# AU-Master-Thesis/magics

Hardware: AMD Instinct MI355X
Metric: GBP iterations/sec (whole node), N robots x K horizon (higher is better)
Workload: dtype f64

## Files before the change

magics_amd/csrc/mgx_sweep.h:

```cpp
#pragma once
#include <hip/hip_runtime.h>

#include "gbp_math.h"
#include "mgx_dev.h"

namespace mgx {

constexpr int SWEEP_BLOCK = 128;
enum { ROLE_DYN = 0, ROLE_UV = 1 };
#ifndef MGX_WIDE
#define MGX_WIDE 0
#endif
template <int KT, bool PERSIST>
constexpr int sweep_waves() { return (MGX_WIDE && PERSIST && KT > 0 && 4 * KT <= 64) ? 4 : 2; }
template <int KT, bool PERSIST>
constexpr int sweep_threads() { return 64 * sweep_waves<KT, PERSIST>(); }

__device__ __forceinline__ void ld_soa4(const double *base, int stride, int item, double (&o)[4]) {
#pragma unroll
    for (int c = 0; c < 4; c++) o[c] = base[(size_t)c * stride + item];
}
__device__ __forceinline__ void ld_soa16(const double *base, int stride, int item, double (&o)[16]) {
#pragma unroll
    for (int c = 0; c < 16; c++) o[c] = base[(size_t)c * stride + item];
// ... 975 lines not shown
        }
        if (internal) {
#pragma unroll
            for (int c = 0; c < 4; c++) s_snap[(20 + c) * K + lane] = mu[c];
        }
    };

    auto quad_core = [&](const double *s_in, double *cov_img, bool &ok, bool &fin, double &mu_q) __attribute__((always_inline)) {
        const int q = lane / K, i = lane - q * K;
        double eta[4], lam[16];
#pragma unroll
        for (int c = 0; c < 4; c++) eta[c] = s_in[c * K + i];
#pragma unroll
        for (int c = 0; c < 16; c++) lam[c] = s_in[(4 + c) * K + i];
        bool not_zero = false;
#pragma unroll
        for (int c = 0; c < 16; c++) not_zero = not_zero || (lam[c] > 1e-6);
        double r0[4], r1[4], r2[4], mn[4], cf[4];
#pragma unroll
        for (int c = 0; c < 4; c++) {
            r0[c] = (q == 0) ? lam[4 + c] : lam[c];
            r1[c] = (q <= 1) ? lam[8 + c] : lam[4 + c];
            r2[c] = (q <= 2) ? lam[12 + c] : lam[8 + c];
        }
        minors_of_removed_row(r0, r1, r2, mn);
#pragma unroll
        for (int j = 0; j < 4; j++) cf[j] = ((q + j) & 1) ? -mn[j] : mn[j];
        const double row0[4] = {lam[0], lam[1], lam[2], lam[3]};
        const double det = __shfl(det_from_row0(row0, cf), i, 64);
        ok = not_zero && det != 0.0;
        const double id = 1.0 / det;
        double col[4];
        bool fin_own = true;
#pragma unroll
        for (int j = 0; j < 4; j++) {
            col[j] = cf[j] * id;
            fin_own = fin_own && std::isfinite(col[j]);
        }
        unsigned long long bad = __ballot(!fin_own);
        constexpr int KS = QUADFIN ? KT : 1;
        bad |= (bad >> KS) | (bad >> (2 * KS)) | (bad >> (3 * KS));
        fin = ((bad >> i) & 1ull) == 0ull;
        if (ok) {
#pragma unroll
            for (int j = 0; j < 4; j++) cov_img[(j * 4 + q) * K + i] = col[j];
            __builtin_amdgcn_wave_barrier();
            if (fin) {
                double cq[4];
#pragma unroll
                for (int c = 0; c < 4; c++) cq[c] = cov_img[(q * 4 + c) * K + i];
                mu_q = ((cq[0] * eta[0] + cq[1] * eta[1]) + cq[2] * eta[2]) + cq[3] * eta[3];
            }
        }
    };
    auto variable_finish_quad = [&](const double *s_in, bool internal) {
        const int q = lane / K, i = lane - q * K;
        double mu_q = s_mu[q * K + i];
        bool ok, fin;
        quad_core(s_in, s_cov, ok, fin, mu_q);
        if (ok) {
            if (fin) s_mu[q * K + i] = mu_q;
            if (q == 0) {
                s_valid[i] = fin ? 1 : 0;
                s_covset[i] = 1;
            }
        }
        if (internal) s_snap[(20 + q) * K + i] = mu_q;
    };
    auto finish = [&](const double *s_in, bool internal) __attribute__((always_inline)) {
        if constexpr (QUADFIN) {
            if (role == ROLE_UV && lane < 4 * K) variable_finish_quad(s_in, internal);
        } else {
            if (is_var) variable_finish(s_in, internal);
        }
    };

    auto dynamic_messages = [&](double *s_out) {
        double me[4], ml[16], oe[4], ol[16];
        const int o = dyn_other_var, oe_ix = dyn_other_edge;
        double paa[4], pab[4], pba[4], pbb[4];
        if (PERSIST) {
            load_dyn_potential(paa, pab, pba, pbb);
        } else {
#pragma unroll
            for (int c = 0; c < 4; c++) { paa[c] = maa[c]; pab[c] = mab[c]; pba[c] = mba[c]; pbb[c] = mbb[c]; }
        }
        if (s_epoch[o] > 0) {
#pragma unroll
            for (int c = 0; c < 4; c++) me[c] = s_snap[c * K + o] - s_fv[c * E1 + oe_ix];
#pragma unroll
            for (int c = 0; c < 16; c++) ml[c] = s_snap[(4 + c) * K + o] - s_fv[(4 + c) * E1 + oe_ix];
        } else {
#pragma unroll
            for (int c = 0; c < 4; c++) me[c] = 0.0;
#pragma unroll
            for (int c = 0; c < 16; c++) ml[c] = 0.0;
        }
        double me2[4], ml2[16];
        const int lane2 = lane + 64;
        const bool has2 = BIG && lane2 < n_dyn;
        if (has2) {
            const int f2 = lane2 % (K - 1), slot2 = lane2 / (K - 1), o2 = f2 + 1 - slot2, oe2 = (1 - slot2) * (K - 1) + f2;
            const bool pres = s_epoch[o2] > 0;
#pragma unroll
            for (int c = 0; c < 4; c++) me2[c] = pres ? s_snap[c * K + o2] - s_fv[c * E1 + oe2] : 0.0;
#pragma unroll
            for (int c = 0; c < 16; c++) ml2[c] = pres ? s_snap[(4 + c) * K + o2] - s_fv[(4 + c) * E1 + oe2] : 0.0;
        }
        if (!dynamic_message(paa, pab, pba, pbb, me, ml, oe, ol)) {
#pragma unroll
            for (int c = 0; c < 4; c++) oe[c] = 0.0;
#pragma unroll
            for (int c = 0; c < 16; c++) ol[c] = 0.0;
        }
#pragma unroll
        for (int c = 0; c < 4; c++) s_out[c * E1 + lane] = oe[c];
#pragma unroll
        for (int c = 0; c < 16; c++) s_out[(4 + c) * E1 + lane] = ol[c];
        if (has2) {
            const int f2 = lane2 % (K - 1), slot2 = lane2 / (K - 1), a2 = 2 * slot2, b2 = 2 * (1 - slot2), it2 = r * (K - 1) + f2;
            double naa[4], nab[4], nba[4], nbb[4];
#pragma unroll
            for (int i = 0; i < 2; i++)
#pragma unroll
                for (int j = 0; j < 2; j++) {
                    naa[i * 2 + j] = w.dyn_m[(size_t)((a2 + i) * 4 + (a2 + j)) * w.ND + it2];
                    nab[i * 2 + j] = w.dyn_m[(size_t)((a2 + i) * 4 + (b2 + j)) * w.ND + it2];
                    nba[i * 2 + j] = w.dyn_m[(size_t)((b2 + i) * 4 + (a2 + j)) * w.ND + it2];
                    nbb[i * 2 + j] = w.dyn_m[(size_t)((b2 + i) * 4 + (b2 + j)) * w.ND + it2];
                }
            if (!dynamic_message(naa, nab, nba, nbb, me2, ml2, oe, ol)) {
#pragma unroll
                for (int c = 0; c < 4; c++) oe[c] = 0.0;
#pragma unroll
                for (int c = 0; c < 16; c++) ol[c] = 0.0;
            }
#pragma unroll
            for (int c = 0; c < 4; c++) s_out[c * E1 + lane2] = oe[c];
#pragma unroll
            for (int c = 0; c < 16; c++) s_out[(4 + c) * E1 + lane2] = ol[c];
        }
    };

    const SdfView sdf = make_sdf_view(w.sdf, w.sdf_w, w.sdf_h, w.world_w, w.world_h);
    auto trk_pad_here = [&]() __attribute__((always_inline)) {
        double p_ = w.trk_pad;
        asm volatile("" : "+v"(p_));
        return p_;
    };
    auto obs_inv_delta_here = [&]() __attribute__((always_inline)) {
        double p_ = w.obs_inv_delta;
        asm volatile("" : "+s"(p_));
        return p_;
    };
    auto unary_messages = [&](uint32_t skip, double *s_out, int itf_gate) __attribute__((always_inline)) {
        if (obs_rows) {
            if (role == ROLE_UF && lane < 4 * (K - 2) && (w.enable & 4u) && !(skip & 4u)) {
                const int j = lane >> 2, q = lane & 3, var = j + 1, col = n_dyn + j;
                double x0[4];
                const bool pres = s_epoch[var] > 0;
#pragma unroll
                for (int c = 0; c < 4; c++) x0[c] = pres ? s_snap[(20 + c) * K + var] : 0.0;
                const long long idx = obstacle_tap(sdf, x0[0], x0[1], w.obs_delta, q);
                const double hq = (idx >= 0) ? sdf_value(w.sdf[idx]) : 0.0;
                double h[4];
#pragma unroll
                for (int t = 0; t < 4; t++) h[t] = __shfl(hq, (lane & ~3) + t, 64);
                double eta_q, lam_q[4];
                obstacle_message_row(h, w.obs_delta, obs_inv_delta_here(), w.inv_s2_obs, x0, q, eta_q, lam_q);
                s_out[q * E1 + col] = eta_q;
#pragma unroll
                for (int c = 0; c < 4; c++) s_out[(4 + q * 4 + c) * E1 + col] = lam_q[c];
            }
        } else if (is_obs && (w.enable & 4u) && !(skip & 4u)) {
            double x0[4], oe[4], ol[16];
            const bool pres = s_epoch[uvar] > 0;
#pragma unroll
            for (int c = 0; c < 4; c++) x0[c] = pres ? s_snap[(20 + c) * K + uvar] : 0.0;
            long long idx[4];
            obstacle_taps(sdf, x0[0], x0[1], w.obs_delta, idx);
            double h[4];
#pragma unroll
            for (int q = 0; q < 4; q++) h[q] = (idx[q] >= 0) ? sdf_value(w.sdf[idx[q]]) : 0.0;
            obstacle_message(h, w.obs_delta, obs_inv_delta_here(), w.inv_s2_obs, x0, oe, ol);
#pragma unroll
            for (int c = 0; c < 4; c++) s_out[c * E1 + uedge] = oe[c];
#pragma unroll
            for (int c = 0; c < 16; c++) s_out[(4 + c) * E1 + uedge] = ol[c];
        }
        if (is_trk && (w.enable & 8u) && itf_gate >= 10 && !(skip & 8u)) {
            double x0[4], oe[4], ol[16];
#pragma unroll
            for (int c = 0; c < 4; c++) x0[c] = s_snap[(20 + c) * K + uvar];
            const int p0 = w.path_ptr[r], np = w.path_ptr[r + 1] - p0;
            if (!tracking_update(w.path_xy + 2 * (size_t)p0, np, trk_pad_here(), w.trk_attr, w.inv_s2_trk, x0, trk_rec,
                                  trk_lp, trk_lv, oe, ol)) {
#pragma unroll
                for (int c = 0; c < 4; c++) oe[c] = 0.0;
#pragma unroll
                for (int c = 0; c < 16; c++) ol[c] = 0.0;
            }
#pragma unroll
            for (int c = 0; c < 4; c++) s_out[c * E1 + uedge] = oe[c];
#pragma unroll
            for (int c = 0; c < 16; c++) s_out[(4 + c) * E1 + uedge] = ol[c];
        }
        if (BIG && role == ROLE_UF && lane + 64 >= K - 2 && lane + 64 < 2 * (K - 2) && (w.enable & 8u) && itf_gate >= 10 &&
            !(skip & 8u)) {
            const int j2 = lane + 64 - (K - 2), var2 = j2 + 1, col2 = n_dyn + (K - 2) + j2, item2 = r * (K - 2) + j2;
            double x0[4], oe[4], ol[16];
#pragma unroll
            for (int c = 0; c < 4; c++) x0[c] = s_snap[(20 + c) * K + var2];
            int rec2 = w.trk_record[item2];
            float lp2[2] = {w.trk_last_pos[item2], w.trk_last_pos[(size_t)w.NT + item2]};
            double lv2 = w.trk_last_val[item2];
            const int p0 = w.path_ptr[r], np = w.path_ptr[r + 1] - p0;
            if (!tracking_update(w.path_xy + 2 * (size_t)p0, np, trk_pad_here(), w.trk_attr, w.inv_s2_trk, x0, rec2, lp2, lv2, oe, ol)) {
#pragma unroll
                for (int c = 0; c < 4; c++) oe[c] = 0.0;
#pragma unroll
                for (int c = 0; c < 16; c++) ol[c] = 0.0;
            }
            w.trk_record[item2] = rec2;
            w.trk_last_pos[item2] = lp2[0];
            w.trk_last_pos[(size_t)w.NT + item2] = lp2[1];
            w.trk_last_val[item2] = lv2;
#pragma unroll
            for (int c = 0; c < 4; c++) s_out[c * E1 + col2] = oe[c];
#pragma unroll
            for (int c = 0; c < 16; c++) s_out[(4 + c) * E1 + col2] = ol[c];
        }
    };

    int my_peer = -1, peer_q0 = 0, peer_q1 = 0;
    bool my_peer_read = false;
    if (PERSIST && radio && ir_on && role == ROLE_UV) {
        peer_q0 = w.peer_ptr[r];
        peer_q1 = w.peer_ptr[r + 1];
        if (peer_q0 + lane < peer_q1) {
            const int pr = w.peer_idx[peer_q0 + lane];
            if (w.antenna[pr] && !w.idle[pr]) my_peer = pr;
        }
        for (int e = w.ir_var_ptr[v0 + 1]; e < w.ir_var_ptr[v0 + 2]; e++) my_peer_read = my_peer_read || w.ir_rec[e].src_robot == my_peer;
    }
    auto progress_of = [&](int pr) __attribute__((always_inline)) {
        if (SHARD && pr >= w.R_local)
            return __hip_atomic_load(&cold().gflag[pr - w.R_local], __ATOMIC_RELAXED, __HIP_MEMORY_SCOPE_SYSTEM);
        return __hip_atomic_load(&w.sweep_flag[pr], __ATOMIC_RELAXED, __HIP_MEMORY_SCOPE_AGENT);
    };
    auto wait_for_progress = [&](unsigned long long want, bool ghosts_only) __attribute__((always_inline)) {
        if (PERSIST && radio && ir_on && role == ROLE_UV) {
            for (int q = peer_q0 + lane; q < peer_q1; q += 64) {
                int pr = my_peer;
                if (q != peer_q0 + lane) {
                    pr = w.peer_idx[q];
                    if (!w.antenna[pr] || w.idle[pr]) pr = -1;
                }
                if (pr < 0 || (ghosts_only && pr < w.R_local)) continue;
                if (!ghosts_only && q == peer_q0 + lane && my_peer_read) continue;
                const long long t0 = wall_clock64();
                unsigned spins = 0;
                while (progress_of(pr) < want) {
                    __builtin_amdgcn_s_sleep(4);
                    if ((++spins & 31u) == 0u) {
                        if (__hip_atomic_load(cold().sweep_abort, __ATOMIC_RELAXED, __HIP_MEMORY_SCOPE_AGENT) != 0ull) break;
                        if (wall_clock64() - t0 > cold_plan().timeout_ticks) {
                            const unsigned long long word = cold_plan().flag_base + 1ull;
                            __hip_atomic_store(cold().sweep_abort, word, __ATOMIC_RELAXED, __HIP_MEMORY_SCOPE_AGENT);
                            __hip_atomic_store(cold().sweep_err, word, __ATOMIC_RELAXED, __HIP_MEMORY_SCOPE_SYSTEM);
                            break;
                        }
                    }
                }
            }
        }
    };
    auto wait_for_peers = [&](int k) __attribute__((always_inline)) { wait_for_progress(plan.flag_base + (unsigned long long)k, false); };
    int xp0 = 0, xp1 = 0;
    if (SHARD && role == ROLE_UV) {
        xp0 = __builtin_amdgcn_readfirstlane(cold().xp_ptr[r]);
        xp1 = __builtin_amdgcn_readfirstlane(cold().xp_ptr[r + 1]);
    }

    bool prefired = false;
    bool par_done = false;
    bool pending = false;
    bool early = false;
    auto adopt_early = [&](int t0, int step) __attribute__((always_inline)) {
        for (int t = t0; t < 20 * E; t += step) {
            const int c = t / E, e = t - c * E;
            s_fv[c * E1 + e] = s_sh[c * E1 + e];
        }
    };
    int last_int_seg = -1, last_ext_seg = -1;
    int kbase = 0;
    if (PLDS && lane == 0) s_ps[0] = 0u;
    if (PLDS) __builtin_amdgcn_wave_barrier();
#ifdef MGX_STAMPS
    unsigned long long c_f = 0, c_fb = 0, c_v = 0, c_vb = 0, t_extf = t_staged, t_extv = t_staged, t_loop0 = t_staged;
    unsigned long long rt0 = __builtin_amdgcn_s_memrealtime();
    unsigned long long p_wait = 0, p_extf = 0, p_extv = 0, p_int = 0, p_pub = 0;
    unsigned long long qs[16] = {0, 0, 0, 0, 0, 0, 0, 0, 0, 0, 0, 0, 0, 0, 0, 0};
#define PSTAMP(v) const unsigned long long v = __builtin_readcyclecounter()
#define QSTAMP(i, since) do { const unsigned long long _n = __builtin_readcyclecounter(); qs[i] += _n - (since); (since) = _n; } while (0)
#define QBEGIN(v) unsigned long long v = __builtin_readcyclecounter()
#else
#define PSTAMP(v)
#define QSTAMP(i, since)
#define QBEGIN(v)
#endif
    for (int k = 0; PLDS || k < nseg; k++) {
        if (k == 0) {
            const int plans_done = PLDS ? (int)ps_word(0) : 0;
            const bool upd_now = PLDS ? plan_dword(1) != 0u : w.upd != nullptr;
            if (upd_now) {
                if constexpr (PLDS) {
#pragma unroll
                    for (int c = 0; c < 4; c++) u_rec[c] = s_urec[c];
                    u_bel = (lane < 20 && role < 2) ? s_tmp[4 * K + role * 20 + lane] : 0.0;
                }
                const double upd_max_speed = PLDS ? reinterpret_cast<const double *>(s_plan + 2 + MAX_SEGS / 2)[0] : w.upd_max_speed;
                const double upd_delta_t = PLDS ? reinterpret_cast<const double *>(s_plan + 2 + MAX_SEGS / 2)[1] : w.upd_delta_t;
                const uint32_t what = (uint32_t)u_rec[3];
                const int i = role == 0 ? K - 1 : 0;
                if (role < 2 && (role == 0 ? (what & 1u) : (what & 2u))) {
                    double m[4];
                    if (role == 0) {
                        const double ex = s_mu[0 * K + i], ey = s_mu[1 * K + i];
                        double hx = u_rec[0] - ex, hy = u_rec[1] - ey;
                        const double dist = std::sqrt(hx * hx + hy * hy);
                        double nx = hx, ny = hy;
                        if (!(dist == 0.0 || std::isinf(dist))) { nx = hx / dist; ny = hy / dist; }
                        const double sp = (upd_max_speed < dist || dist != dist) ? upd_max_speed : dist;
                        const double vx = sp * nx, vy = sp * ny;
                        m[0] = ex + vx * upd_delta_t; m[1] = ey + vy * upd_delta_t; m[2] = vx; m[3] = vy;
                    } else {
        #pragma unroll
                        for (int c = 0; c < 4; c++) {
                            const double m0 = s_mu[c * K + 0], m1 = s_mu[c * K + 1];
                            m[c] = m0 + u_rec[2] * (m1 - m0);
                        }
                    }
                    __builtin_amdgcn_wave_barrier();
                    if (lane < 4) {
                        double pl[4];
        #pragma unroll
                        for (int c = 0; c < 4; c++) pl[c] = s_prior[(4 + lane * 4 + c) * K + i];
                        const double pe = ((pl[0] * m[0] + pl[1] * m[1]) + pl[2] * m[2]) + pl[3] * m[3];
                        s_prior[lane * K + i] = pe;
                        blob[L.prior() + lane * K + i] = pe;
                    } else if (lane < 8) {
                        const double mc = lane == 4 ? m[0] : (lane == 5 ? m[1] : (lane == 6 ? m[2] : m[3]));
                        s_mu[(lane - 4) * K + i] = mc;
                        s_snap[(20 + lane - 4) * K + i] = mc;
                        if (PERSIST && have_xmu) s_xmu[(lane - 4) * K + i] = mc;
                    } else if (lane == 8) {
                        s_epoch[i] += 1;
                    }
                    if (lane < 20) s_snap[lane * K + i] = u_bel;
                    const int es[4] = {(i >= 1) ? (K - 1) + (i - 1) : -1, (i <= K - 2) ? i : -1,
                                       (i >= 1 && i <= K - 2) ? n_dyn + (i - 1) : -1, (i >= 1 && i <= K - 2) ? n_dyn + (K - 2) + (i - 1) : -1};
                    for (int t = lane; t < 80; t += 64) {
                        const int col = es[t & 3];
                        if (col >= 0) {
                            s_fv[(t >> 2) * E1 + col] = 0.0;
                            if (PERSIST) s_sh[(t >> 2) * E1 + col] = 0.0;
                        }
                    }
                    if (HAS_IR) {
                        const int x0 = w.ir_var_ptr[v0 + i], x1 = w.ir_var_ptr[v0 + i + 1];
                        for (int e = x0 + lane; e < x1; e += 64) {
                            if (w.enable & 2u) {
        #pragma unroll
                                for (int c = 0; c < 4; c++) w.ir_bmu[(size_t)c * w.NI + e] = m[c];
                            }
                            w.ir_fv_eta[0 * (size_t)w.NI + e] = 0.0;
                            w.ir_fv_eta[1 * (size_t)w.NI + e] = 0.0;
                            w.ir_fv_lam[0 * (size_t)w.NI + e] = 0.0;
                            w.ir_fv_lam[1 * (size_t)w.NI + e] = 0.0;
                            w.ir_fv_lam[4 * (size_t)w.NI + e] = 0.0;
                            w.ir_fv_lam[5 * (size_t)w.NI + e] = 0.0;
                            if (STAGE_IR) {
        #pragma unroll
                                for (int c = 0; c < 6; c++) s_ir[(e - ie0) * IR_STRIDE + c] = 0.0;
                            }
                        }
                    }
                }
                __syncthreads();
            }
            if (PERSIST && plans_done == 0) {
                for (int t = tid; t < 20 * E1; t += NT) s_sh[t] = s_fv[t];
                __syncthreads();
            }
            my_epoch = (sum_t < 4 * K) ? s_epoch[sum_t % K] : 0u;
            if constexpr (PLDS) {
                nseg = (int)plan_dword(0);
                const int q = lane & (MAX_SEGS - 1), q1 = (q + 1) & (MAX_SEGS - 1);
                auto byte_of = [&](int base, int i) __attribute__((always_inline)) { return (s_plan[base + (i >> 2)] >> (8 * (i & 3))) & 0xffu; };
                const uint32_t e_q = byte_of(2, q), n_q = byte_of(2 + MAX_SEGS / 4, q);
                const uint32_t e_1 = q + 1 < MAX_SEGS ? byte_of(2, q1) : 0u, n_1 = q + 1 < MAX_SEGS ? byte_of(2 + MAX_SEGS / 4, q1) : 0u;
                const bool in = lane < nseg;
                const unsigned long long m_int = __ballot(in && n_q > 0u), m_ext = __ballot(in && e_q != 0u);
                last_int_seg = m_int ? 63 - __clzll((long long)m_int) : -1;
                last_ext_seg = m_ext ? 63 - __clzll((long long)m_ext) : -1;
                has_int_var = m_int != 0ull && !idle;
                any_sweep = has_int_var || (m_ext != 0ull && radio);
                kbase = plans_done ? (int)ps_word(1) - 1 : 0;
                const bool lingers = LINGER && census && plan.linger_ticks > 0;
                if (lane < MAX_SEGS) {
                    const uint32_t bits = (e_q ? SEG_EXT : 0u) | (lane == nseg - 1 ? SEG_LAST : 0u) | (lane == last_int_seg ? SEG_LAST_INT : 0u) |
                                          (lane == last_ext_seg ? SEG_LAST_EXT : 0u) | ((lane == 0 && plans_done == 0) ? SEG_FIRST_OF_LAUNCH : 0u) |
                                          (lingers ? SEG_LINGERS : 0u);
                    s_seg[lane] = uint2{bits | (n_q << 8) | ((e_1 ? 1u : 0u) << 16) | (n_1 << 24), (uint32_t)(kbase + lane)};
                }
                __builtin_amdgcn_wave_barrier();
                if (lane == 0) {
                    s_ps[1] = (uint32_t)(kbase + nseg);
                    s_ps[2] = (has_int_var ? 1u : 0u) | (any_sweep ? 2u : 0u);
                }
                __builtin_amdgcn_wave_barrier();
            } else if (PERSIST) {
                bool plan_int = false, plan_has_ext = false;
                last_int_seg = last_ext_seg = -1;
                for (int q = 0; q < nseg; q++) {
                    if (plan_n_int(q) > 0) { plan_int = true; last_int_seg = q; }
                    if (plan_ext(q)) { plan_has_ext = true; last_ext_seg = q; }
                }
                has_int_var = plan_int && !idle;
                any_sweep = has_int_var || (plan_has_ext && radio);
            }
        }
        uint32_t seg_b = 0u;
        int kg = k;
        if constexpr (PLDS) {
            const uint2 e = s_seg[k];
            seg_b = (uint32_t)__builtin_amdgcn_readfirstlane((int)e.x);
            kg = __builtin_amdgcn_readfirstlane((int)e.y);
        } else if (PERSIST) {
            seg_b = (plan_ext(k) ? SEG_EXT : 0u) | ((uint32_t)plan_n_int(k) << 8) | (k == nseg - 1 ? SEG_LAST : 0u) | (k == last_int_seg ? SEG_LAST_INT : 0u) |
                    (k == last_ext_seg ? SEG_LAST_EXT : 0u) | (k == 0 ? SEG_FIRST_OF_LAUNCH : 0u);
            if (k + 1 < nseg) seg_b |= ((plan_ext(k + 1) ? 1u : 0u) << 16) | ((uint32_t)plan_n_int(k + 1) << 24);
        }
        const bool is_last_int_seg = (seg_b & SEG_LAST_INT) != 0u, is_last_ext_seg = (seg_b & SEG_LAST_EXT) != 0u;
        const bool lingers = LINGER && (seg_b & SEG_LINGERS) != 0u;
        if (PERSIST) asm volatile("" : "+v"(tid), "+v"(lane), "+v"(my_j), "+v"(pf_dst));
        const uint32_t ext_k = PERSIST ? ((seg_b & SEG_EXT) ? (PH_EXT_FACTOR | PH_EXT_VARIABLE) : 0u) : ext_mask;
        const uint32_t int_k = PERSIST ? (PH_INT_FACTOR | PH_INT_VARIABLE) : int_mask;
        const int n_int_k = PERSIST ? (int)((seg_b >> 8) & 0xffu) : n_int;
        const bool last_seg = PERSIST ? (seg_b & SEG_LAST) != 0u : true;
        PSTAMP(ps0);
        QBEGIN(qt);
        if (PERSIST && ext_k && k > 0) {
            wait_for_peers(kg);
            QSTAMP(0, qt);
            if (!(FUSED && par_done)) __syncthreads();
            QSTAMP(1, qt);
        }
        PSTAMP(ps1);
        if (ext_k & PH_EXT_FACTOR) {
            external_factor_sweep(k, kg, !PERSIST || is_last_ext_seg);
            QSTAMP(2, qt);
            __syncthreads();
            QSTAMP(3, qt);
        }
        PSTAMP(ps2);
#ifdef MGX_STAMPS
        if (k == 0) t_extf = __builtin_readcyclecounter();
#endif
        prefired = false;
        if constexpr (FUSED) {
            par_done = (ext_k & PH_EXT_VARIABLE) && radio && early && n_int_k == 1;
            if (par_done) {
                const bool is_last = is_last_int_seg && last_seg;
                const int q = lane / K, i = lane - q * K;
                bool ok_i = false, fin_i = false;
                double mu_i = 0.0;
                if (role == ROLE_UV) {
                    double *t_ = s_fv;
                    s_fv = s_sh;
                    s_sh = t_;
                    variable_sums(s_snap, true, false);
                    QSTAMP(4, qt);
                    if (lane < 4 * K) quad_core(s_snap, s_cov, ok_i, fin_i, mu_i);
                } else {
                    if (role == ROLE_DYN && lane < 4 * K) {
                        variable_sums_from(lane, 4 * K, s_tmp, false, false);
                        QSTAMP(4, qt);
                        double mu_x = s_mu[q * K + i];
                        bool ok_x, fin_x;
                        quad_core(s_tmp, s_tmp + 4 * K, ok_x, fin_x, mu_x);
                        s_xmu[q * K + i] = mu_x - 0.0;
                        if (q == 0) s_xok[i] = (ok_x ? 1 : 0) | (fin_x ? 2 : 0);
                    }
                    double *t_ = s_fv;
                    s_fv = s_sh;
                    s_sh = t_;
                }
                QSTAMP(6, qt);
                __syncthreads();
                QSTAMP(7, qt);
                DELAY_AT(5, true);
                if (role == ROLE_UV && lane < 4 * K) {
                    double mu_fin = mu_i;
                    const int xs = s_xok[i];
                    if (!(ok_i && fin_i)) {
                        mu_fin = s_xmu[q * K + i];
                        if (!ok_i && (xs & 1)) {
#pragma unroll
                            for (int j = 0; j < 4; j++) s_cov[(j * 4 + q) * K + i] = s_tmp[(4 + j * 4 + q) * K + i];
                        }
                    }
                    s_mu[q * K + i] = mu_fin;
                    s_snap[(20 + q) * K + i] = mu_fin;
                    if (is_last) {
                        s_prior[q * K + i] = s_snap[q * K + i];
#pragma unroll
                        for (int c = 0; c < 4; c++) s_prior[(4 + q * 4 + c) * K + i] = s_snap[(4 + q * 4 + c) * K + i];
                    }
                    if (q == 0) {
                        if (ok_i) {
                            s_valid[i] = fin_i ? 1 : 0;
                            s_covset[i] = 1;
                        } else if (xs & 1) {
                            s_valid[i] = (xs & 2) ? 1 : 0;
                            s_covset[i] = 1;
                        }
                    }
                }
                if (ir_on && (!is_last_ext_seg || lingers)) have_xmu = true;
                if (ir_on && is_last_ext_seg) {
                    for (int q = tid; q < ne; q += NT) {
                        const int e = ie0 + (q == tid ? my_j : edge_of_lane(q));
                        int dst;
                        if (q == tid) {
                            if (!pf_gate) continue;
                            dst = pf_dst;
                        } else {
                            if (!w.ir_gate[e]) continue;
                            dst = w.ir_rec[e].dst;
                        }
                        const int iv = dst & 0xffff;
#pragma unroll
                        for (int c = 0; c < 4; c++) w.ir_bmu[(size_t)c * w.NI + e] = s_xmu[c * K + iv];
                    }
                }
                if (is_last) __syncthreads();
                itf += 1;
                early = false;
            } else if ((ext_k & PH_EXT_VARIABLE) && radio) {
                const bool ext_is_last = last_seg && n_int_k == 0;
                double *s_sum = ext_is_last ? s_prior : s_tmp;
                prefired = !early && n_int_k > 0 && !idle && (int_k & PH_INT_FACTOR) && skip0 == 0u;
                const bool keep_means = ir_on && (!is_last_ext_seg || lingers);
                if (role == ROLE_UV) {
                    variable_sums(s_sum, false, false);
                    QSTAMP(4, qt);
                    finish(s_sum, false);
                    if (keep_means && lane < 4 * K) s_xmu[lane] = s_mu[lane] - 0.0;
                }
                if (prefired && (NW == 4 || role == ROLE_UV)) unary_messages(0u, s_sh, itf);
                if (prefired && is_dyn && (w.enable & 1u)) dynamic_messages(s_sh);
                QSTAMP(6, qt);
                if (keep_means) have_xmu = true;
                if (ir_on && is_last_ext_seg) {
                    __syncthreads();
                    for (int q = tid; q < ne; q += NT) {
                        const int e = ie0 + (q == tid ? my_j : edge_of_lane(q));
                        int dst;
                        if (q == tid) {
                            if (!pf_gate) continue;
                            dst = pf_dst;
                        } else {
                            if (!w.ir_gate[e]) continue;
                            dst = w.ir_rec[e].dst;
                        }
                        const int i = dst & 0xffff;
#pragma unroll
                        for (int c = 0; c < 4; c++) w.ir_bmu[(size_t)c * w.NI + e] = s_mu[c * K + i] - 0.0;
                    }
                }
                if (prefired) __syncthreads();
            }
            if (early || prefired) {
                double *t_ = s_fv;
                s_fv = s_sh;
                s_sh = t_;
            }
        } else if (ext_k & PH_EXT_VARIABLE) {
            const bool ext_is_last = PERSIST ? (last_seg && n_int_k == 0) : !has_int_var;
            double *s_sum = ext_is_last ? s_prior : s_tmp;
            if (radio) variable_sums(s_sum, false, false);
            QSTAMP(4, qt);
            __syncthreads();
            QSTAMP(5, qt);
            prefired = !early && radio && n_int_k > 0 && !idle && (int_k & PH_INT_FACTOR) && skip0 == 0u;
            if (prefired && is_dyn && (w.enable & 1u)) dynamic_messages(s_fv);
            if (PERSIST && early && radio && role == ROLE_DYN) adopt_early(lane, 64);
            if (radio && is_var) variable_finish(s_sum, false);
            if (prefired) unary_messages(0u, s_fv, itf);
            QSTAMP(6, qt);
            __syncthreads();
            QSTAMP(7, qt);
            if (PERSIST && radio && ir_on && (!is_last_ext_seg || lingers)) {
                if (tid < 4 * K) s_xmu[tid] = s_mu[tid] - 0.0;
                have_xmu = true;
            }
            if (radio && ir_on && (!PERSIST || is_last_ext_seg)) {
                for (int q = tid; q < ne; q += NT) {
                    const int e = ie0 + (q == tid ? my_j : edge_of_lane(q));
                    int dst;
                    if (q == tid && (do_extf || PERSIST)) {
                        if (!pf_gate) continue;
                        dst = pf_dst;
                    } else {
                        if (!w.ir_gate[e]) continue;
                        dst = w.ir_rec[e].dst;
                    }
                    const int i = dst & 0xffff;
#pragma unroll
                    for (int c = 0; c < 4; c++) w.ir_bmu[(size_t)c * w.NI + e] = s_mu[c * K + i] - 0.0;
                }
            }
        }
        QSTAMP(8, qt);
        PSTAMP(ps3);
#ifdef MGX_STAMPS
        if (k == 0) { t_extv = __builtin_readcyclecounter(); t_loop0 = t_extv; rt0 = __builtin_amdgcn_s_memrealtime(); }
#endif
        if (PERSIST && !FUSED && early && !((ext_k & PH_EXT_VARIABLE) && radio)) {
            adopt_early(tid, NT);
            __syncthreads();
        }
        if (PERSIST && early) prefired = true;
        early = false;
        for (int it = 0; it < n_int_k && !idle && !par_done; it++) {
            asm volatile("" : "+v"(tid), "+v"(lane));
            STAMP(t0);
            if ((int_k & PH_INT_FACTOR) && it == 0 && prefired) {
                itf += 1;
            } else if (int_k & PH_INT_FACTOR) {
                if (is_dyn && (w.enable & 1u) && !(it == 0 && (skip0 & 1u))) dynamic_messages(s_fv);
                if (pending) {
                    finish(s_snap, true);
                    if (NW == 4) __syncthreads();
                }
                pending = false;
                unary_messages(it == 0 ? skip0 : 0u, s_fv, itf);
                itf += 1;
                STAMP(t1);
                __syncthreads();
                STAMP(t2);
                STAMP_ADD(c_f, t0, t1);
                STAMP_ADD(c_fb, t1, t2);
            }
            STAMP(t3);
            if (int_k & PH_INT_VARIABLE) {
                const bool is_last = it == n_int_k - 1 && (!PERSIST || (is_last_int_seg && (last_seg || !radio)));
                variable_sums(s_snap, true, is_last);
                pending = true;
                STAMP(t4);
                __syncthreads();
                STAMP(t5);
                STAMP_ADD(c_v, t3, t4);
                STAMP_ADD(c_vb, t4, t5);
            }
        }
        if (census && !CENSUS_EARLY && (seg_b & SEG_FIRST_OF_LAUNCH)) {
            const unsigned long long v = tid == 0 ? __hip_atomic_load(cold().decision, __ATOMIC_RELAXED, __HIP_MEMORY_SCOPE_AGENT) : 0ull;
            if (census_says_abort(v)) return;
        }
        PSTAMP(ps4);
        if (PERSIST && !last_seg) {
            QSTAMP(9, qt);
            if (role == ROLE_UV && pending) finish(s_snap, true);
            if (NW == 4) __syncthreads();
            const int ob = (w.cur + kg + 1) & 1;
            const unsigned long long next_count = plan.flag_base + (unsigned long long)kg + 1ull;
            auto chunk_of = [&](int t, uint32_t seq) __attribute__((always_inline)) {
                const int ch = t / K, i = t - ch * K, da = (3 * ch) >> 1;
                v4u32 v;
#ifdef MGX_XREC_CHECKSUM
                if (ch == XREC_CHUNKS - 1) {
                    unsigned x = s_epoch[i];
                    for (int n = 0; n < 22; n++) { const double f = s_snap[n * K + i]; x ^= (unsigned)__double2loint(f) ^ (unsigned)__double2hiint(f); }
                    v.x = x; v.y = (unsigned)(r * 64 + i); v.z = 0u; v.w = seq;
                    return v;
                }
#endif
                const double A = s_snap[da * K + i], B = s_snap[(da + 1) * K + i];
                v.x = (ch & 1) ? (unsigned)__double2hiint(A) : (unsigned)__double2loint(A);
                v.y = (ch & 1) ? (unsigned)__double2loint(B) : (unsigned)__double2hiint(A);
                v.z = (ch & 1) ? (unsigned)__double2hiint(B) : (unsigned)__double2loint(B);
                if (3 * ch + 2 == XREC_EPOCH_DWORD) v.z = s_epoch[i];
                v.w = seq;
                return v;
            };
            const unsigned xbase = (unsigned)v0 * (unsigned)XREC_BYTES;
            if (role == ROLE_UV) {
                QSTAMP(10, qt);
                __builtin_amdgcn_wave_barrier();
                DELAY_AT(1, true);
                TLSTAMP(k, 0);
                {
                    const uint32_t seq = xrec_seq(next_count);
                    for (int t = lane; t < XREC_CHUNKS * K; t += 64) st16_agent_raw(rs_x, xbase + 16u * (unsigned)t, ob ? xrec_bytes : 0u, chunk_of(t, seq));
                }
                QSTAMP(11, qt);
                DELAY_AT(2, true);
                TLSTAMP(k, 1);
                if (lane == 0) __hip_atomic_store(&w.sweep_flag[r], next_count, __ATOMIC_RELAXED, __HIP_MEMORY_SCOPE_AGENT);
                QSTAMP(12, qt);
                if (SHARD && xp1 > xp0) {
                    if (k == 0) wait_for_progress(plan.flag_base, true);
                    for (int t = xp0; t < xp1; t++) {
                        const XPushRec xr = cold().xp_rec[t];
                        const __amdgpu_buffer_rsrc_t rs_peer = uniform_rsrc(ob ? xr.xrec[1] : xr.xrec[0], (unsigned)K * (unsigned)XREC_BYTES);
                        const uint32_t seq = xrec_seq(next_count + xr.flag_delta);
                        for (int t2 = lane; t2 < XREC_CHUNKS * K; t2 += 64) {
                            v4u32 c = chunk_of(t2, seq);
                            c.w ^= xrec_mix(c.x, c.y, c.z);
                            st16_system_raw(rs_peer, 16u * (unsigned)t2, c);
                        }
                        if (lane == 0)
                            __hip_atomic_store(reinterpret_cast<unsigned long long *>(xr.flag), next_count + xr.flag_delta, __ATOMIC_RELAXED,
                                               __HIP_MEMORY_SCOPE_SYSTEM);
                    }
                }
            }
            pending = false;
            early = (seg_b >> 24) > 0u && !idle && skip0 == 0u;
            DELAY_AT(3, role == ROLE_DYN);
            if (early) {
                if (is_dyn && (w.enable & 1u)) dynamic_messages(s_sh);
                unary_messages(0u, s_sh, itf + ((((seg_b >> 16) & 1u) && radio) ? 1 : 0));
            }
            QSTAMP(13, qt);
        }
#ifdef MGX_STAMPS
        {
            PSTAMP(ps5);
            p_wait += ps1 - ps0; p_extf += ps2 - ps1; p_extv += ps3 - ps2; p_int += ps4 - ps3; p_pub += ps5 - ps4;
        }
#endif
        if constexpr (PLDS) {
            if (last_seg && !lingers) break;
        }
        if constexpr (LINGER) {
            if (last_seg) {
                const int plans_done = (int)ps_word(0);
                any_sweep = (ps_word(2) & 2u) != 0u;
                int *s_verdict = reinterpret_cast<int *>(lds + 1);
                const unsigned long long number = cold_plan().launch_seq + (unsigned long long)plans_done + 1ull;
                if (role == 0) {
                    const unsigned long long cur2 = 2ull * (number - 1ull);
                    unsigned long long *go = cold_plan().linger_go;
                    const uint32_t seq = xrec_seq(number);
                    const unsigned char *dslot = cold_plan().linger_dev + (size_t)(number & 1ull) * cold_plan().linger_dev_stride;
                    const __amdgpu_buffer_rsrc_t rs_s = sc1_rsrc(dslot, LINGER_SLOT_HEAD + LINGER_UPD_BYTES * (unsigned)w.R_local);
                    const unsigned my_off = lane < 8 ? 16u * (unsigned)lane : LINGER_SLOT_HEAD + LINGER_UPD_BYTES * (unsigned)r + 16u * (unsigned)(lane < 11 ? lane - 8 : 0);
                    v4u32 c = v4u32{0u, 0u, 0u, 0u};
                    unsigned long long gw = 0ull;
                    int verdict = -1;
                    long long t0 = 0;
                    for (unsigned spins = 0; verdict < 0; spins++) {
                        if (lane < 11) c = ld16_agent_raw(rs_s, my_off);
                        else if (lane == 11) gw = __hip_atomic_load(go, __ATOMIC_RELAXED, __HIP_MEMORY_SCOPE_AGENT);
                        const unsigned long long ok = __ballot(lane < 11 && c.w == seq);
                        const uint32_t has_upd = (uint32_t)__builtin_amdgcn_readlane((int)c.y, 0);
                        unsigned long long g = ((unsigned long long)(uint32_t)__builtin_amdgcn_readlane((int)(gw >> 32), 11) << 32) |
                                               (uint32_t)__builtin_amdgcn_readlane((int)(gw & 0xffffffffull), 11);
                        if ((ok & 0xffull) == 0xffull && (!has_upd || (ok & 0x700ull) == 0x700ull)) { verdict = 1; break; }
                        if (g == cur2 + 1ull) { verdict = 0; break; }
                        if (spins == 0u) t0 = wall_clock64();
                        if (spins < 8u) __builtin_amdgcn_s_sleep(2);
                        else __builtin_amdgcn_s_sleep(24);
                        if ((spins & 7u) == 7u && g <= cur2 &&
                            (__hip_atomic_load(cold().sweep_abort, __ATOMIC_RELAXED, __HIP_MEMORY_SCOPE_AGENT) != 0ull || wall_clock64() - t0 > cold_plan().linger_ticks)) {
                            unsigned long long old = 0ull;
                            if (lane == 11) old = __hip_atomic_fetch_max(go, cur2 + 1ull, __ATOMIC_RELAXED, __HIP_MEMORY_SCOPE_AGENT);
                            g = ((unsigned long long)(uint32_t)__builtin_amdgcn_readlane((int)(old >> 32), 11) << 32) | (uint32_t)__builtin_amdgcn_readlane((int)(old & 0xffffffffull), 11);
                            if (g <= cur2 + 1ull) { verdict = 0; break; }
                        }
                    }
                    if (verdict == 1) {
                        if (lane < 8) { s_plan[3 * lane] = c.x; s_plan[3 * lane + 1] = c.y; s_plan[3 * lane + 2] = c.z; }
                        else if (lane < 11) {
                            uint32_t *u = reinterpret_cast<uint32_t *>(s_urec) + 3 * (lane - 8);
                            u[0] = c.x; u[1] = c.y;
                            if (lane < 10) u[2] = c.z;
                        }
                    }
                    if (lane == 0) *s_verdict = verdict;
                }
                if (role == ROLE_UV && pending) finish(s_snap, true);
                pending = false;
                __syncthreads();
                const int iu = role == 0 ? K - 1 : 0;
                if (lane < 20 && role < 2) s_tmp[4 * K + role * 20 + lane] = any_sweep ? s_prior[lane * K + iu] : blob[L.bel() + lane * K + iu];
                if (role == ROLE_DYN && any_sweep) copy_words_wave(blob + L.bel(), s_prior, 20 * K, lane);
                StageRegs<(KT > 0 ? 20 * KT : 2), NT> r_prior;
                if constexpr (KT > 0) r_prior.load(blob + L.prior(), tid);
                __syncthreads();
                if (*s_verdict != 1) break;
                if (lane == 0) s_ps[0] = (uint32_t)(plans_done + 1);
                {
                    if constexpr (KT > 0) r_prior.store(s_prior, tid);
                    else copy_words(s_prior, blob + L.prior(), 20 * K, tid, NT);
                    __syncthreads();
                    if (tid == 0) __hip_atomic_store(&cold().census[blockIdx.x], number, __ATOMIC_RELAXED, __HIP_MEMORY_SCOPE_AGENT);
                }
                k = -1;
            }
        }
    }
    int total_segs = nseg;
    if constexpr (PLDS) {
        total_segs = (int)ps_word(1);
        any_sweep = (ps_word(2) & 2u) != 0u;
    }
    {
        if (role == ROLE_UV) {
            if (pending) finish(s_snap, true);
        } else if (role == ROLE_DYN) {
            copy_words_wave(blob + L.fv(), s_fv, 20 * E1, lane);
            if (any_sweep && !bel_dead) copy_words_wave(blob + L.bel(), s_prior, 20 * K, lane);
        }
        __syncthreads();
#ifdef MGX_STAMPS
        if (w.dbg && lane == 0 && role < 2) {
            unsigned long long *d = w.dbg + ((size_t)blockIdx.x * 2 + role) * 8;
            d[0] = c_f; d[1] = c_fb; d[2] = c_v; d[3] = c_vb; d[4] = __builtin_readcyclecounter() - t_loop0;
            d[5] = __builtin_amdgcn_s_memrealtime() - rt0;
            d[6] = t_staged - t_k0;
            d[0] = (d[0] & 0xffffffffull) | ((t_extf - t_staged) << 32);
            d[1] = (d[1] & 0xffffffffull) | ((t_extv - t_extf) << 32);
            if (PERSIST) {
                d[0] = p_wait; d[1] = p_extf; d[2] = p_extv; d[3] = p_int; d[4] = p_pub;
                unsigned long long *d2 = w.dbg + (size_t)((census ? gridDim.x - 1 : gridDim.x) + 4) * 16 + ((size_t)blockIdx.x * 2 + role) * 16;
                for (int i = 0; i < 16; i++) d2[i] = qs[i];
                d2[14] = q_arrive;
            }
        }
#endif
    }
    if (PERSIST) snap_out = (w.cur + total_segs) & 1;
    if (SHARD && role == ROLE_UV && lane == 0) {
        for (int t = xp0; t < xp1; t++) {
            const XPushRec xr = cold().xp_rec[t];
            __hip_atomic_store(reinterpret_cast<unsigned long long *>(xr.flag), plan.flag_base + xr.flag_delta + (unsigned long long)total_segs,
                               __ATOMIC_RELAXED, __HIP_MEMORY_SCOPE_SYSTEM);
        }
    }

    for (int t = tid; t < 16 * K; t += NT)
        if (s_covset[t % K]) blob[L.cov() + t] = s_cov[t];
    copy_words(blob + L.mu(), s_mu, 4 * K, tid, NT);
    copy_words(blob + L.valid(), (const double *)s_valid, K, tid, NT);
    if (snap_out >= 0) {
        double *dst = w.snap[snap_out] + (size_t)v0 * SNAP_W;
        for (int t = tid; t < SNAP_W * K; t += NT) dst[t] = s_snap[(t % SNAP_W) * K + (t / SNAP_W)];
        for (int t = tid; t < K; t += NT) w.snap_epoch[snap_out][v0 + t] = s_epoch[t];
    }
    if (is_trk) {
        w.trk_record[trk_item] = trk_rec;
        w.trk_last_pos[trk_item] = trk_lp[0];
        w.trk_last_pos[(size_t)w.NT + trk_item] = trk_lp[1];
        w.trk_last_val[trk_item] = trk_lv;
    }
    if (tid == 0) w.iter_factor[r] = itf;
#ifdef MGX_STAMPS
    if (w.dbg && lane == 0 && role < 2) w.dbg[((size_t)blockIdx.x * 2 + role) * 8 + 7] = __builtin_readcyclecounter() - t_k0;
#endif
}

}
```

Baseline: 125,900.

## Write belief directly at linger boundary and drop prior restage barrier

In lingering persistent mode, the final variable sums no longer overwrite s_prior. Instead, belief is written to global memory directly from the last ext or int segment, and flags in s_ps[2] record which segment was last. This lets the plan-boundary code skip reloading the prior from global through registers, along with one of its __syncthreads. The aim is to cut per-plan boundary latency in the persistent loop, at the risk of subtle correctness issues in the belief/prior handoff. Optional boundary timing stamps are also added under a compile flag.

```diff
diff --git a/magics_amd/csrc/mgx_sweep.h b/magics_amd/csrc/mgx_sweep.h
--- a/magics_amd/csrc/mgx_sweep.h
+++ b/magics_amd/csrc/mgx_sweep.h
@@ -1301,16 +1301,25 @@
     unsigned long long p_wait = 0, p_extf = 0, p_extv = 0, p_int = 0, p_pub = 0;
     unsigned long long qs[16] = {0, 0, 0, 0, 0, 0, 0, 0, 0, 0, 0, 0, 0, 0, 0, 0};
 #define PSTAMP(v) const unsigned long long v = __builtin_readcyclecounter()
-#define QSTAMP(i, since) do { const unsigned long long _n = __builtin_readcyclecounter(); qs[i] += _n - (since); (since) = _n; } while (0)
+#define QSTAMP_(i, since) do { const unsigned long long _n = __builtin_readcyclecounter(); qs[i] += _n - (since); (since) = _n; } while (0)
 #define QBEGIN(v) unsigned long long v = __builtin_readcyclecounter()
+#ifdef MGX_STAMPS_BOUNDARY
+#define QSTAMP(i, since)
+#define BSTAMP(i, since) QSTAMP_(i, since)
+#else
+#define QSTAMP(i, since) QSTAMP_(i, since)
+#define BSTAMP(i, since)
+#endif
 #else
 #define PSTAMP(v)
 #define QSTAMP(i, since)
+#define BSTAMP(i, since)
 #define QBEGIN(v)
 #endif
     for (int k = 0; PLDS || k < nseg; k++) {
         if (k == 0) {
             const int plans_done = PLDS ? (int)ps_word(0) : 0;
+            QBEGIN(bq);
             const bool upd_now = PLDS ? plan_dword(1) != 0u : w.upd != nullptr;
             if (upd_now) {
                 if constexpr (PLDS) {
@@ -1414,9 +1423,11 @@
                     s_seg[lane] = uint2{bits | (n_q << 8) | ((e_1 ? 1u : 0u) << 16) | (n_1 << 24), (uint32_t)(kbase + lane)};
                 }
                 __builtin_amdgcn_wave_barrier();
+                const bool tail_int = last_int_seg == nseg - 1;
                 if (lane == 0) {
                     s_ps[1] = (uint32_t)(kbase + nseg);
-                    s_ps[2] = (has_int_var ? 1u : 0u) | (any_sweep ? 2u : 0u);
+                    s_ps[2] = (has_int_var ? 1u : 0u) | (any_sweep ? 2u : 0u) |
+                              ((radio && !tail_int && last_ext_seg == nseg - 1) ? 4u : 0u) | ((has_int_var && (!radio || tail_int)) ? 8u : 0u);
                 }
                 __builtin_amdgcn_wave_barrier();
             } else if (PERSIST) {
@@ -1429,6 +1440,7 @@
                 has_int_var = plan_int && !idle;
                 any_sweep = has_int_var || (plan_has_ext && radio);
             }
+            if (plans_done > 0) { BSTAMP(3, bq); }
         }
         uint32_t seg_b = 0u;
         int kg = k;
@@ -1512,7 +1524,7 @@
                     }
                     s_mu[q * K + i] = mu_fin;
                     s_snap[(20 + q) * K + i] = mu_fin;
-                    if (is_last) {
+                    if (is_last && !lingers) {
                         s_prior[q * K + i] = s_snap[q * K + i];
 #pragma unroll
                         for (int c = 0; c < 4; c++) s_prior[(4 + q * 4 + c) * K + i] = s_snap[(4 + q * 4 + c) * K + i];
@@ -1544,18 +1556,25 @@
                         for (int c = 0; c < 4; c++) w.ir_bmu[(size_t)c * w.NI + e] = s_xmu[c * K + iv];
                     }
                 }
-                if (is_last) __syncthreads();
+                if (is_last && !lingers) __syncthreads();
                 itf += 1;
                 early = false;
             } else if ((ext_k & PH_EXT_VARIABLE) && radio) {
                 const bool ext_is_last = last_seg && n_int_k == 0;
-                double *s_sum = ext_is_last ? s_prior : s_tmp;
+                double *s_sum = (ext_is_last && !lingers) ? s_prior : s_tmp;
                 prefired = !early && n_int_k > 0 && !idle && (int_k & PH_INT_FACTOR) && skip0 == 0u;
                 const bool keep_means = ir_on && (!is_last_ext_seg || lingers);
                 if (role == ROLE_UV) {
                     variable_sums(s_sum, false, false);
                     QSTAMP(4, qt);
                     finish(s_sum, false);
+                    if (ext_is_last && lingers) {
+                        copy_words_wave(blob + L.bel(), s_tmp, 20 * K, lane);
+                        const int pc = lane < 20 ? lane : lane - 20;
+                        const double stale = lane < 40 ? s_sum[pc * K + (lane < 20 ? K - 1 : 0)] : 0.0;
+                        __builtin_amdgcn_wave_barrier();
+                        if (lane < 40) s_tmp[4 * K + lane] = stale;
+                    }
                     if (keep_means && lane < 4 * K) s_xmu[lane] = s_mu[lane] - 0.0;
                 }
                 if (prefired && (NW == 4 || role == ROLE_UV)) unary_messages(0u, s_sh, itf);
@@ -1588,7 +1607,7 @@
             }
         } else if (ext_k & PH_EXT_VARIABLE) {
             const bool ext_is_last = PERSIST ? (last_seg && n_int_k == 0) : !has_int_var;
-            double *s_sum = ext_is_last ? s_prior : s_tmp;
+            double *s_sum = (ext_is_last && !lingers) ? s_prior : s_tmp;
             if (radio) variable_sums(s_sum, false, false);
             QSTAMP(4, qt);
             __syncthreads();
@@ -1601,6 +1620,13 @@
             QSTAMP(6, qt);
             __syncthreads();
             QSTAMP(7, qt);
+            if (LINGER && radio && ext_is_last && lingers) {
+                copy_words(blob + L.bel(), s_sum, 20 * K, tid, NT);
+                const int pc = tid < 20 ? tid : tid - 20;
+                const double stale = tid < 40 ? s_sum[pc * K + (tid < 20 ? K - 1 : 0)] : 0.0;
+                __syncthreads();
+                if (tid < 40) s_tmp[4 * K + tid] = stale;
+            }
             if (PERSIST && radio && ir_on && (!is_last_ext_seg || lingers)) {
                 if (tid < 4 * K) s_xmu[tid] = s_mu[tid] - 0.0;
                 have_xmu = true;
@@ -1652,11 +1678,14 @@
                 STAMP(t2);
                 STAMP_ADD(c_f, t0, t1);
                 STAMP_ADD(c_fb, t1, t2);
+#ifdef MGX_STAMPS_BOUNDARY
+                if (PLDS && k == 0 && it == 0 && ps_word(0) > 0u) { qs[4] += t1 - t0; qs[5] += t2 - t1; }
+#endif
             }
             STAMP(t3);
             if (int_k & PH_INT_VARIABLE) {
                 const bool is_last = it == n_int_k - 1 && (!PERSIST || (is_last_int_seg && (last_seg || !radio)));
-                variable_sums(s_snap, true, is_last);
+                variable_sums(s_snap, true, is_last && !lingers);
                 pending = true;
                 STAMP(t4);
                 __syncthreads();
@@ -1750,6 +1779,10 @@
                 const int plans_done = (int)ps_word(0);
                 any_sweep = (ps_word(2) & 2u) != 0u;
                 int *s_verdict = reinterpret_cast<int *>(lds + 1);
+                if (!any_sweep) __syncthreads();
+#ifdef MGX_STAMPS_BOUNDARY
+                const unsigned long long b_t0 = __builtin_readcyclecounter();
+#endif
                 const unsigned long long number = cold_plan().launch_seq + (unsigned long long)plans_done + 1ull;
                 if (role == 0) {
                     const unsigned long long cur2 = 2ull * (number - 1ull);
@@ -1794,21 +1827,27 @@
                 }
                 if (role == ROLE_UV && pending) finish(s_snap, true);
                 pending = false;
+#ifdef MGX_STAMPS_BOUNDARY
+                const unsigned long long b_t1 = __builtin_readcyclecounter();
+#endif
                 __syncthreads();
+#ifdef MGX_STAMPS_BOUNDARY
+                unsigned long long b_t2 = __builtin_readcyclecounter();
+#endif
+                const bool ext_last = (ps_word(2) & 4u) != 0u, int_last = (ps_word(2) & 8u) != 0u;
+                if (any_sweep && !ext_last && role == ROLE_DYN) copy_words_wave(blob + L.bel(), int_last ? s_snap : s_prior, 20 * K, lane);
+                if (*s_verdict != 1) break;
                 const int iu = role == 0 ? K - 1 : 0;
-                if (lane < 20 && role < 2) s_tmp[4 * K + role * 20 + lane] = any_sweep ? s_prior[lane * K + iu] : blob[L.bel() + lane * K + iu];
-                if (role == ROLE_DYN && any_sweep) copy_words_wave(blob + L.bel(), s_prior, 20 * K, lane);
-                StageRegs<(KT > 0 ? 20 * KT : 2), NT> r_prior;
-                if constexpr (KT > 0) r_prior.load(blob + L.prior(), tid);
-                __syncthreads();
-                if (*s_verdict != 1) break;
+                if (!ext_last && lane < 20 && role < 2)
+                    s_tmp[4 * K + role * 20 + lane] = int_last ? s_snap[lane * K + iu] : (any_sweep ? s_prior[lane * K + iu] : blob[L.bel() + lane * K + iu]);
                 if (lane == 0) s_ps[0] = (uint32_t)(plans_done + 1);
-                {
-                    if constexpr (KT > 0) r_prior.store(s_prior, tid);
-                    else copy_words(s_prior, blob + L.prior(), 20 * K, tid, NT);
-                    __syncthreads();
-                    if (tid == 0) __hip_atomic_store(&cold().census[blockIdx.x], number, __ATOMIC_RELAXED, __HIP_MEMORY_SCOPE_AGENT);
-                }
+                if (tid == 0) __hip_atomic_store(&cold().census[blockIdx.x], number, __ATOMIC_RELAXED, __HIP_MEMORY_SCOPE_AGENT);
+#ifdef MGX_STAMPS_BOUNDARY
+                qs[0] += b_t1 - b_t0;
+                qs[1] += b_t2 - b_t1;
+                BSTAMP(2, b_t2);
+                qs[6] += 1ull;
+#endif
                 k = -1;
             }
         }
@@ -1823,7 +1862,8 @@
             if (pending) finish(s_snap, true);
         } else if (role == ROLE_DYN) {
             copy_words_wave(blob + L.fv(), s_fv, 20 * E1, lane);
-            if (any_sweep && !bel_dead) copy_words_wave(blob + L.bel(), s_prior, 20 * K, lane);
+            const bool lingered = LINGER && census && plan.linger_ticks > 0;
+            if (any_sweep && !bel_dead && !lingered) copy_words_wave(blob + L.bel(), s_prior, 20 * K, lane);
         }
         __syncthreads();
 #ifdef MGX_STAMPS
```

New measurement: 126,500, median of 6. Within noise of the previous version (+0.5%).
